# HikariTJU/LD

Measured on AMD Instinct MI355X. Metric: images/sec (1333x800) GFocal-R50<-R101 LD train step, higher is better.
Workload: dtype f32

## Files before the change

include/ld_hip.h:

```cpp
#ifndef LD_HIP_H_
#define LD_HIP_H_

#include <stddef.h>
#include <stdint.h>

#ifdef __cplusplus
extern "C" {
#endif

#define LD_MAX_LEVELS 8
#define LD_NUM_LOSS_KEYS 8

#define LD_EINVAL (-1)
#define LD_ENOSPACE (-2)
#define LD_EUNSUPPORTED (-3)

typedef void* ld_stream_t;

typedef struct {
  int32_t H, W;
  int32_t stride;
  int32_t offset;
} ld_level_t;

// ... 205 lines not shown
  void* y_raw_c8;
} ld_conv_epilogue_t;

size_t ld_conv_weight_image_floats(int Cout, int Cin, int KH, int KW,
                                   int backward);
int ld_conv_weight_transform(const float* w, int Cout, int Cin, int KH, int KW,
                             float* wt_fwd, float* wt_bwd, ld_stream_t stream);
typedef struct {
  const float* w;
  float* wt_fwd;
  float* wt_bwd;
  int32_t Cout, Cin, ntaps, first_block;
} ld_wt_job_t;
int ld_conv_weight_transform_batch(const ld_wt_job_t* jobs, const int32_t* block_job,
                                   int nblocks, ld_stream_t stream);
int ld_conv_weight_transform_tiles(int Cout, int Cin, int ntaps, int bf16);
int ld_conv_weight_transform_batch_tiled(const ld_wt_job_t* jobs,
                                         const int32_t* block_job, int nblocks, int bf16,
                                         ld_stream_t stream);
int ld_conv_forward(const ld_conv_t* c, const float* x, const float* wt_fwd,
                    const ld_conv_epilogue_t* ep, float* y, ld_stream_t stream);
int ld_conv_dgrad(const ld_conv_t* c, const float* dy, const float* wt_bwd,
                  float* dx, ld_stream_t stream);
int ld_conv_dgrad_acc(const ld_conv_t* c, const float* dy, const float* wt_bwd,
                      const float* addend, float* dx, ld_stream_t stream);
int ld_conv_tune_forward(const ld_conv_t* c, const float* x, const float* wt_fwd,
                         const ld_conv_epilogue_t* ep, float* y,
                         ld_stream_t stream);
int ld_conv_tune_dgrad(const ld_conv_t* c, const float* dy, const float* wt_bwd,
                       float* dx, ld_stream_t stream);
int ld_conv_tune_load(const char* path);
int ld_conv_tune_save(const char* path);
int ld_conv_tune_clear(void);
long long ld_conv_tune_hits(const int* key);
int ld_conv_tune_reset_hits(void);
size_t ld_conv_wgrad_workspace_bytes(const ld_conv_t* c);
size_t ld_conv_tune_wgrad_workspace_bytes(const ld_conv_t* c);
int ld_conv_wgrad(const ld_conv_t* c, const float* x, const float* dy, float* dw,
                  int accumulate, void* workspace, size_t workspace_bytes,
                  ld_stream_t stream);
typedef struct {
  const float* slabs;
  float* dw;
  int32_t splits, ntaps, Cout, Cin, accumulate, first_block;
} ld_wgrad_job_t;
int ld_conv_wgrad_partial(const ld_conv_t* c, int family, const void* x, const void* dy,
                          void* slabs, size_t slab_bytes, ld_wgrad_job_t* job,
                          ld_stream_t stream);
int ld_wgrad_reduce_batch(const ld_wgrad_job_t* jobs, const int32_t* block_job,
                          int nblocks, ld_stream_t stream);
int ld_conv_wgrad_plan(const ld_conv_t* c, int* out);
int ld_conv_tune_wgrad(const ld_conv_t* c, const float* x, const float* dy, float* dw,
                       void* workspace, size_t workspace_bytes, ld_stream_t stream);

size_t ld_conv_bf16_weight_image_elems(int Cout, int Cin, int KH, int KW,
                                       int backward);
int ld_conv_bf16_weight_transform(const float* w, int Cout, int Cin, int KH, int KW,
                                  void* wt_fwd, void* wt_bwd, ld_stream_t stream);
int ld_conv_bf16_weight_transform_batch(const ld_wt_job_t* jobs,
                                        const int32_t* block_job, int nblocks,
                                        ld_stream_t stream);
int ld_conv_bf16_forward(const ld_conv_t* c, const float* x, const void* wt_fwd,
                         const ld_conv_epilogue_t* ep, float* y, ld_stream_t stream);
int ld_conv_bf16_tune_forward(const ld_conv_t* c, const float* x, const void* wt_fwd,
                              const ld_conv_epilogue_t* ep, float* y,
                              ld_stream_t stream);
// ... 459 lines not shown
```

ld_amd/csrc/conv.hip:

```cpp
#include <hip/hip_runtime.h>
#include <type_traits>
#include <stdio.h>
#include <stdlib.h>

#include <mutex>
#include <string>
#include <unordered_map>
#include <vector>

#include "conv_common.h"
#include "conv_tune.h"

namespace {

template <int BM, int BNT, int BKT, int MODE, int KG, int WVM, int WVN>
__global__ __launch_bounds__(64 * WVM * WVN * KG) void conv_igemm_kernel(ConvK a) {
  constexpr int NT = 64 * WVM * WVN;
  constexpr int WM = BM / WVM, WN = BNT / WVN;
  constexpr int TM = WM / 32, TN = WN / 32;
  constexpr int A_PER = BKT * BM / NT;
  constexpr int B_PER = BKT * BNT / NT;
  static_assert(A_PER >= 1 && B_PER >= 1, "tile too small");
  constexpr int NBUF = 2;
  constexpr int GROUP_LDS = NBUF * BKT * (BM + BNT);
  constexpr int NACC = TM * TN * 16;
  static_assert(KG == 1 || (KG - 1) * NACC * NT <= KG * GROUP_LDS,
                "split-K reduction does not fit the tile LDS");
  __shared__ float lds[KG * GROUP_LDS + 2 * BM];
  const int kg = __builtin_amdgcn_readfirstlane((int)threadIdx.x / NT);
  float* As = lds + kg * GROUP_LDS;
  float* Bs = As + NBUF * BKT * BM;

  const int t = threadIdx.x % NT, lane = t & 63, wave = t >> 6;
  const int wm = wave / WVN, wn = wave % WVN;
  const int mtiles = (a.Cout + BM - 1) / BM;
  const int tile = xcd_swizzle(blockIdx.x, gridDim.x);
  const int m0 = (tile % mtiles) * BM;
// ... 276 lines not shown
      locate_out(a.g, p, l, hc, wc);
      p = a.foff[l] + (2 * hc + a.ph) * a.fW[l] + 2 * wc + a.pw;
      prow = a.Pfull;
    }
    const size_t colbase = (size_t)n * a.Cout * prow + p;
#pragma unroll
    for (int i = 0; i < TM; ++i) {
      const int rbase = wm * WM + i * 32 + 4 * lk;
      float res[16];
      if (has_res) {
#pragma unroll
        for (int r = 0; r < 16; ++r) {
          const int row = rbase + (r & 3) + 8 * (r >> 2);
          res[r] = (m0 + row < a.Cout)
                       ? a.residual[colbase + (size_t)(m0 + row) * prow]
                       : 0.0f;
        }
      }
#pragma unroll
      for (int r = 0; r < 16; ++r) {
        const int row = rbase + (r & 3) + 8 * (r >> 2);
        if (m0 + row >= a.Cout) continue;
        float v = acc[i][j][r] * s_scale[row] + s_shift[row];
        if (MODE == 0 && a.y_raw)
          a.y_raw[colbase + (size_t)(m0 + row) * prow] = acc[i][j][r];
        if (has_res) v += res[r];
        if (relu) v = fmaxf(v, 0.0f);
        a.y[colbase + (size_t)(m0 + row) * prow] = v;
      }
    }
  }
}

template <int TM, int TN, int WVM, int MODE, int D, int OCC, int KS, int DBG = 0>
__global__ __launch_bounds__(256, OCC) void conv_stream_kernel(ConvK a) {
  static_assert(KS == 1 || (KS == 4 && WVM == 1), "KS is 1 or 4");
  static_assert(D * (TM + TN) < 64, "ring exceeds the 6-bit vmcnt counter");
  constexpr int WVN = 4 / WVM;
  constexpr int WM = TM * 32, WN = TN * 32;
  constexpr int BM = KS == 4 ? WM : WVM * WM, BNT = KS == 4 ? WN : WVN * WN;
  __shared__ float red[KS == 4 ? 2 * TM * TN * 16 * 64 : 1];
  const int lane = threadIdx.x & 63;
  const int wave = __builtin_amdgcn_readfirstlane((int)threadIdx.x >> 6);
  const int wm = KS == 4 ? 0 : wave / WVN, wn = KS == 4 ? 0 : wave % WVN;
  const int kslice = KS == 4 ? wave : 0;
  const int l31 = lane & 31, lk = lane >> 5;
  const int mtiles = (a.Cout + BM - 1) / BM;
  const int tile = xcd_swizzle(blockIdx.x, gridDim.x);
  const int m0 = (tile % mtiles) * BM + wm * WM;
  const int n0 = (tile / mtiles) * BNT + wn * WN;
  if (m0 >= a.Cout || n0 >= a.J) return;

  const int Cin = __builtin_amdgcn_readfirstlane(a.Cin);
  const int Cout = __builtin_amdgcn_readfirstlane(a.Cout);
  const int KW = __builtin_amdgcn_readfirstlane(a.KW);
  const int Pin = __builtin_amdgcn_readfirstlane(a.Pin);
  const int Kpad = __builtin_amdgcn_readfirstlane(a.Kpad);
  const int ntw = __builtin_amdgcn_readfirstlane(MODE == 1 ? a.ntw : a.KW);
  const int ntaps = __builtin_amdgcn_readfirstlane(
      MODE == 1 ? a.nth * a.ntw : a.KH * a.KW);

  int bHin[TN], bWin[TN], boff[TN], bh0[TN], bw0[TN];
#pragma unroll
  for (int j = 0; j < TN; ++j) {
    const int jb = n0 + j * 32 + l31;
    bHin[j] = 0;
    bWin[j] = 0;
    boff[j] = 0;
    bh0[j] = 0;
    bw0[j] = 0;
    if (jb < a.J) {
      const int n = jb / a.Pout, p = jb - n * a.Pout;
      int bl, bho, bwo;
      locate_out(a.g, p, bl, bho, bwo);
      bHin[j] = a.g.lv[bl].Hin;
      bWin[j] = a.g.lv[bl].Win;
      boff[j] = n * Cin * Pin + a.g.lv[bl].off_in + lk * Pin;
      if (MODE == 1) {
        bh0[j] = bho + a.ch0;
        bw0[j] = bwo + a.cw0;
      } else {
        bh0[j] = bho * a.g.stride - a.g.pad;
        bw0[j] = bwo * a.g.stride - a.g.pad;
// ... 185 lines not shown
            rv[j][e] = buf_load(r_res, ok ? voff[j] : kOOB, (unsigned)(rl + e) * prow4);
          }
      }
#pragma unroll
      for (int e = 0; e < 4; ++e) {
        const bool ok = m0 + 4 * lk + rl + e < Cout;
        const float scale = has_aff ? sc[e] : 1.0f;
        const float shift = sh[e] + bi[e];
        const unsigned so = (unsigned)(rl + e) * prow4;
#pragma unroll
        for (int j = 0; j < TN; ++j) {
          const int r = 4 * g + e;
          const unsigned vo = ok ? voff[j] : kOOB;
          const float av = acc[i][j][r];
          float v = av * scale + shift;
          if (RAW)
            __builtin_amdgcn_raw_buffer_store_b32(__builtin_bit_cast(unsigned, av), r_raw,
                                                  vo, so, 0);
          if (RES) v += rv[j][e];
          v = relu ? fmaxf(v, 0.0f) : v;
          __builtin_amdgcn_raw_buffer_store_b32(__builtin_bit_cast(unsigned, v), r_y, vo,
                                                so, 0);
        }
      }
    }
  };
  if (has_res) {
    if (has_raw) run(std::true_type{}, std::true_type{});
    else run(std::true_type{}, std::false_type{});
  } else {
    if (has_raw) run(std::false_type{}, std::true_type{});
    else run(std::false_type{}, std::false_type{});
  }
}

template <int VEC>
struct VecF;
template <>
struct VecF<2> { typedef float T __attribute__((ext_vector_type(2))); };
template <>
struct VecF<4> { typedef float T __attribute__((ext_vector_type(4))); };

template <int VEC>
__device__ __forceinline__ typename VecF<VEC>::T buf_load_vec(rsrc_t r, unsigned voff,
                                                             unsigned soff) {
  typedef typename VecF<VEC>::T V;
  if constexpr (VEC == 2)
    return __builtin_bit_cast(V, __builtin_amdgcn_raw_buffer_load_b64(r, voff, soff, 0));
  else
    return __builtin_bit_cast(V, __builtin_amdgcn_raw_buffer_load_b128(r, voff, soff, 0));
}

template <int TM, int VEC, int WVM, int D>
__global__ __launch_bounds__(256, 2) void conv1x1_vec_kernel(ConvK a) {
  static_assert(D * (TM + 1) < 64, "ring exceeds the 6-bit vmcnt counter");
  typedef typename VecF<VEC>::T V;
  constexpr int WVN = 4 / WVM;
  constexpr int WM = TM * 32, WN = VEC * 32;
  constexpr int BM = WVM * WM, BNT = WVN * WN;
  const int lane = threadIdx.x & 63;
  const int wave = __builtin_amdgcn_readfirstlane((int)threadIdx.x >> 6);
  const int wm = wave / WVN, wn = wave % WVN;
  const int l31 = lane & 31, lk = lane >> 5;
  const int mtiles = (a.Cout + BM - 1) / BM;
  const int tile = xcd_swizzle(blockIdx.x, gridDim.x);
  const int m0 = (tile % mtiles) * BM + wm * WM;
// ... 925 lines not shown
  }
  return LD_EUNSUPPORTED;
}

#define MODE1_TAPS(k) ((k).nth > 0 ? (k).nth * (k).ntw : (k).KH * (k).KW)
inline bool stream_cfg_fits(const ConvK& k, const StreamCfg& c) {
  if (c.wvm < 1) return false;
  if (k.Cin % (2 * c.d) != 0) return false;
  if (c.ks == 2) {
    if (k.KH != 1 || k.KW != 1 || k.g.stride != 1 || k.g.pad != 0 || k.nth > 0 ||
        k.Pin != k.Pout || k.Pout % c.tn != 0 || k.x_c8 || k.y_c8 || k.res_c8)
      return false;
    const uintptr_t m = (uintptr_t)(c.tn * 4 - 1);
    if ((((uintptr_t)k.x | (uintptr_t)k.y | (uintptr_t)k.residual |
          (uintptr_t)k.y_raw) & m) != 0)
      return false;
    const int bmv = c.wvm * c.tm * 32, cout32v = (k.Cout + 31) / 32 * 32;
    if (c.wvm > 1 && bmv > cout32v) return false;
    if (c.wvm == 1 && c.tm * 32 >= cout32v + 32) return false;
    return true;
  }
  if (c.d == 4 && k.Cin % 16 == 0) return false;
  const int bm = c.wvm * c.tm * 32;
  const int cout32 = (k.Cout + 31) / 32 * 32;
  if (c.ks == 4) {
    const int nchunks = (MODE1_TAPS(k)) * (k.Cin / (2 * c.d));
    if (nchunks < 16) return false;
  }
  if (c.wvm > 1 && bm > cout32) return false;
  if (c.wvm == 1 && c.tm * 32 >= cout32 + 32) return false;
  return true;
}

inline int stream_cfg_model(const ConvK& k) {
  int best = -1;
  double best_t = 0;
  for (int i = 0; i < kNumStreamCfgs; ++i) {
    const StreamCfg& c = kStreamCfgs[i];
    if (c.ks == 2) continue;
    if (!stream_cfg_fits(k, c)) continue;
    const int bm = (c.ks == 4 ? 1 : c.wvm) * c.tm * 32;
    const int bn = (c.ks == 4 ? 1 : 4 / c.wvm) * c.tn * 32;
    const long nb = (long)((k.Cout + bm - 1) / bm) * ((k.J + bn - 1) / bn);
    const int area = c.tm * c.tn;
    const double eff = (area >= 4 ? 0.90 : area >= 2 ? 0.84 : 0.79) *
                       (c.ks == 4 ? 0.97 : 1.0);
    const int occ = area >= 4 ? 4 : 5;
    const double rounds =
        nb <= 256L * occ ? (double)((nb + 255) / 256) : (double)nb / 256.0;
    const double t = rounds * (c.ks == 4 ? 1 : 4) * area / eff;
    if (best < 0 || t < best_t) {
      best = i;
      best_t = t;
    }
  }
  return best;
}

inline LdTuneCfg stream_cfg_rec(const StreamCfg& c) {
  return LdTuneCfg{c.tm, c.tn, c.wvm, c.d, c.ks};
}

template <int MODE>
int launch_stream(const ConvK& k, hipStream_t stream) {
  if (k.Cin % 8 != 0) return LD_EUNSUPPORTED;
  auto launch = [&](const StreamCfg& c, int cap) {
    return launch_stream_cfg<MODE>(k, c, stream, cap);
  };
  auto by_model = [&] {
    const int m = stream_cfg_model(k);
    return m < 0 ? LD_EUNSUPPORTED : launch(kStreamCfgs[m], 0);
  };
  auto forced = [&](int* rc) {
    const char* env = getenv("LD_CONV_STREAM");
    if (!env) return false;
    *rc = LD_EUNSUPPORTED;
    if (env[0] == '0' && env[1] == 0) return true;
    StreamCfg c;
    c.ks = 1;
    int cap = 0;
    if (sscanf(env, "%dx%dx%dx%dx%dx%d", &c.tm, &c.tn, &c.wvm, &c.d, &c.ks, &cap) < 4)
      return false;
    while (c.d > 4 && k.Cin % (2 * c.d) != 0) c.d /= 2;
    if (!(c.ks == 2 && !stream_cfg_fits(k, c))) {
      *rc = launch(c, cap);
      if (*rc != LD_EUNSUPPORTED) return true;
      c.ks = 1;
      *rc = launch(c, cap);
      if (*rc != LD_EUNSUPPORTED) return true;
    }
    *rc = by_model();
    return true;
  };
  return launch_picked(MODE, 0, k, kStreamCfgs, forced, stream_cfg_rec, stream_cfg_fits,
                       stream_cfg_model, launch);
}

template <int MODE>
int tune_stream(const ConvK& k, hipStream_t stream) {
  if (k.Cin % 8 != 0) return 1;
  const LdTuneKey key = make_tune_key(MODE, 0, k);
  if (int r = tune_refused(key, stream)) return r;
  int pick = stream_cfg_model(k);
  if (pick < 0) return 1;
  TuneTimer timer(stream);
  float best_ms = -1.0f;
  int best_cap = 0;
  static const int kCaps[] = {0, 4, 3, 2};
  for (int i = 0; i < kNumStreamCfgs; ++i) {
    if (!stream_cfg_fits(k, kStreamCfgs[i])) continue;
    for (const int cap_try : kCaps) {
      const float ms = timer.time(
          [&] { return launch_stream_cfg<MODE>(k, kStreamCfgs[i], stream, cap_try); });
      if (ms == TuneTimer::kLaunchFailed) break;
      if (ms < 0.0f) continue;
      if (best_ms < 0.0f || ms < best_ms * (cap_try ? 0.99f : 1.0f)) {
        best_ms = ms;
        pick = i;
        best_cap = cap_try;
      }
    }
  }
  const StreamCfg& c = kStreamCfgs[pick];
  if (tune_log_level() == 1) {
    const double fl = 2.0 * k.J * k.Cout * k.Cin *
                      (MODE == 1 ? k.nth * k.ntw : k.KH * k.KW);
    fprintf(stderr,
            "[ld_conv] mode %d Cin %d Cout %d k %dx%d s%d J %d lv %d -> "
            "%dx%dx%dx%dx%d cap %d  %.1f TFLOP/s\n",
            MODE, k.Cin, k.Cout, k.KH, k.KW, k.g.stride, k.J, k.g.num_levels,
            c.tm, c.tn, c.wvm, c.d, c.ks, best_cap, tune_tflops(fl, best_ms));
  }
  if (best_ms > 0.0f) {
    LdTuneCfg rec = stream_cfg_rec(c);
    rec.cap = best_cap;
    ld_tune_store(key, rec);
  }
  return 0;
}

template <int MODE>
int launch_igemm(const ConvK& k_in, hipStream_t stream) {
  ConvK k = k_in;
  k.pipe = 1;
  if (const char* env = getenv("LD_CONV_PIPE")) k.pipe = atoi(env) != 0;
  if constexpr (MODE != 2) {
    const int rc = launch_stream<MODE>(k, stream);
    if (rc != LD_EUNSUPPORTED) return rc;
  }
  const TileCfg c = pick_tile(k);
  const int nb = tile_blocks(k, c);
  int kgroups = 1;
  if (c.bm == 64 && c.bn == 64 && MODE != 2) {
    const int ksteps = ((k.Cin + c.bk - 1) / c.bk) * k.KH * k.KW;
    if (nb < 400 && ksteps >= 8) kgroups = 2;
// ... 79 lines not shown
  if (g_tune.find(k) == g_tune.end()) return -1;
  auto it = g_tune_hits.find(k);
  return it == g_tune_hits.end() ? 0 : it->second;
}

extern "C" int ld_conv_tune_reset_hits(void) {
  std::lock_guard<std::mutex> lock(g_tune_mu);
  g_tune_hits.clear();
  return 0;
}

void ld_tune_store(const LdTuneKey& key, const LdTuneCfg& cfg) {
  std::lock_guard<std::mutex> lock(g_tune_mu);
  g_tune[key] = cfg;
}

extern "C" int ld_conv_tune_load(const char* path) {
  if (!path || !*path) return LD_EINVAL;
  FILE* f = fopen(path, "r");
  if (!f) return LD_EINVAL;
  int n = 0;
  char line[1024];
  while (fgets(line, sizeof(line), f)) {
    if (line[0] == '#' || line[0] == '\n') continue;
    LdTuneKey k;
    LdTuneCfg c;
    int pos = 0, adv = 0, got = 0;
    for (int i = 0; i < 18; ++i)
      if (sscanf(line + pos, "%d%n", &k.v[i], &adv) == 1) {
        pos += adv;
        ++got;
      }
    c.cap = 0;
    if (got == 18 && sscanf(line + pos, "%d %d %d %d %d %d", &c.tm, &c.tn, &c.wvm, &c.d,
                            &c.ks, &c.cap) >= 5) {
      ld_tune_store(k, c);
      ++n;
    }
  }
  fclose(f);
  return n;
}

extern "C" int ld_conv_tune_save(const char* path) {
  if (!path || !*path) return LD_EINVAL;
  FILE* f = fopen(path, "w");
  if (!f) return LD_EINVAL;
  std::lock_guard<std::mutex> lock(g_tune_mu);
  fprintf(f, "# ld_amd conv shape table: MODE Cin Cout KH KW stride pad J levels Hin0 "
             "Win0 ph pw relu res affine family 0 | tm tn wvm d ks cap\n");
  for (const auto& kv : g_tune) {
    for (int i = 0; i < 18; ++i) fprintf(f, "%d ", kv.first.v[i]);
    fprintf(f, " %d %d %d %d %d %d\n", kv.second.tm, kv.second.tn, kv.second.wvm,
            kv.second.d, kv.second.ks, kv.second.cap);
  }
  fclose(f);
  return (int)g_tune.size();
}

extern "C" int ld_conv_tune_clear(void) {
  std::lock_guard<std::mutex> lock(g_tune_mu);
  g_tune.clear();
  return 0;
}

extern "C" size_t ld_conv_weight_image_floats(int Cout, int Cin, int KH, int KW,
                                             int backward) {
  if (Cout < 1 || Cin < 1 || KH < 1 || KW < 1) return 0;
  return backward ? (size_t)KH * KW * kpad_rows(Cout) * Cin
                  : (size_t)KH * KW * kpad_rows(Cin) * Cout;
}

extern "C" int ld_conv_weight_transform(const float* w, int Cout, int Cin, int KH,
                                        int KW, float* wt_fwd, float* wt_bwd,
                                        ld_stream_t stream) {
  if (!w || Cout < 1 || Cin < 1 || KH < 1 || KW < 1 || (!wt_fwd && !wt_bwd))
    return LD_EINVAL;
  const int cip = kpad_rows(Cin), cop = kpad_rows(Cout);
  size_t total = 0;
  if (wt_fwd) total = (size_t)KH * KW * cip * Cout;
  if (wt_bwd) total = max(total, (size_t)KH * KW * cop * Cin);
  LD_LAUNCH(conv_weight_transform_kernel,
                     dim3((unsigned)((total + 255) / 256)), dim3(256), 0,
                     (hipStream_t)stream, w, Cout, Cin, KH * KW, cip, cop, wt_fwd,
                     wt_bwd);
  return (int)hipGetLastError();
}

extern "C" int ld_conv_weight_transform_batch(const ld_wt_job_t* jobs,
                                              const int32_t* block_job, int nblocks,
                                              ld_stream_t stream) {
  if (!jobs || !block_job || nblocks < 1) return LD_EINVAL;
  LD_LAUNCH(conv_weight_transform_batch_kernel, dim3(nblocks), dim3(256), 0,
                     (hipStream_t)stream, jobs, block_job);
  return (int)hipGetLastError();
// ... 763 lines not shown
```

ld_amd/csrc/conv_common.h:

```cpp
#pragma once
#include <hip/hip_runtime.h>
#include <stdint.h>

#include "../../include/ld_hip.h"
#include "ld_launch.h"

struct Geo {
  int stride, pad, num_levels;
  ld_conv_level_t lv[LD_MAX_LEVELS];
};

struct ConvK {
  const float* x;
  const float* wt;
  float* y;
  const float* bias;
  const float* scale;
  const float* shift;
  const float* residual;
  int relu;
  int N, Cin, Cout, KH, KW;
  int Pin, Pout;
  int J;
  int Kpad;
// ... 89 lines not shown
    if (i < a.num_levels && p >= a.lv[i].off_out) l = i;
  const int r = p - a.lv[l].off_out;
  ho = r / a.lv[l].Wout;
  wo = r - ho * a.lv[l].Wout;
}

template <int MODE>
__device__ __forceinline__ bool tap_offset(const Geo& a, int l, int ho, int wo,
                                           int kh, int kw, int& off) {
  const int Hin = a.lv[l].Hin, Win = a.lv[l].Win;
  int hi, wi;
  if (MODE == 0) {
    hi = ho * a.stride - a.pad + kh;
    wi = wo * a.stride - a.pad + kw;
  } else {
    const int hn = ho - a.pad + kh, wn = wo - a.pad + kw;
    if ((hn | wn) < 0 || ((hn | wn) & 1)) return false;
    hi = hn >> 1;
    wi = wn >> 1;
  }
  if (hi < 0 || hi >= Hin || wi < 0 || wi >= Win) return false;
  off = a.lv[l].off_in + hi * Win + wi;
  return true;
}

}

struct LdTuneKey {
  int v[18];
};
struct LdTuneCfg {
  int tm, tn, wvm, d, ks;
  int cap = 0;
};
bool ld_tune_lookup(const LdTuneKey& key, LdTuneCfg* out);
void ld_tune_store(const LdTuneKey& key, const LdTuneCfg& cfg);

namespace {
inline LdTuneKey make_tune_key(int mode, int family, const ConvK& k) {
  static const bool resc8 = [] {
    const char* e = getenv("LD_TUNE_KEY_RESC8");
    return !(e && e[0] == '0');
  }();
  const bool res = k.residual != nullptr || (resc8 && k.res_c8 != nullptr);
  return LdTuneKey{{mode, k.Cin, k.Cout, k.KH, k.KW, k.g.stride, k.g.pad, k.J,
                    k.g.num_levels, k.g.lv[0].Hin, k.g.lv[0].Win, k.ph, k.pw, k.relu,
                    res && !k.tune_plain, k.scale != nullptr, family, 0}};
}
}
```

ld_amd/csrc/conv_tune.h:

```cpp
#pragma once
#include <stdlib.h>

#include "conv_common.h"

namespace {
constexpr int kTuneReps = 3;

inline int tune_log_level() {
  const char* lg = getenv("LD_CONV_TUNE_LOG");
  return lg && (lg[0] == '1' || lg[0] == '2') ? lg[0] - '0' : 0;
}

inline double tune_tflops(double flop, float best_ms) {
  return best_ms > 0 ? flop / (best_ms * 1e-3 / kTuneReps) / 1e12 : 0.0;
}

inline int tune_refused(const LdTuneKey& key, hipStream_t stream) {
  LdTuneCfg have;
  if (ld_tune_lookup(key, &have)) return 1;
  hipStreamCaptureStatus cap = hipStreamCaptureStatusNone;
  (void)hipStreamIsCapturing(stream, &cap);
  return cap != hipStreamCaptureStatusNone ? LD_EUNSUPPORTED : 0;
}

class TuneTimer {
 public:
  static constexpr float kLaunchFailed = -2.0f;

  explicit TuneTimer(hipStream_t stream) : stream_(stream) {
    (void)hipDeviceSynchronize();
    (void)hipEventCreate(&e0_);
    (void)hipEventCreate(&e1_);
  }
  ~TuneTimer() {
// ... 14 lines not shown
      (void)hipEventElapsedTime(&t, e0_, e1_);
      if (ms < 0.0f || t < ms) ms = t;
    }
    return ms;
  }

 private:
  hipStream_t stream_;
  hipEvent_t e0_, e1_;
};

template <class Cfg, int N, class Rec>
int tune_cfg_index(const Cfg (&tab)[N], const LdTuneCfg& t, Rec rec, bool cap_is_shape) {
  for (int i = 0; i < N; ++i) {
    const LdTuneCfg r = rec(tab[i]);
    if (r.tm == t.tm && r.tn == t.tn && r.wvm == t.wvm && r.d == t.d && r.ks == t.ks &&
        (!cap_is_shape || r.cap == t.cap))
      return i;
  }
  return -1;
}

template <class Cfg, int N, class Forced, class Rec, class Fits, class Model, class Launch>
int launch_picked(int mode, int family, const ConvK& k, const Cfg (&tab)[N], Forced forced,
                  Rec rec, Fits fits, Model model, Launch launch) {
  int rc = 0;
  if (forced(&rc)) return rc;
  int pick = -1;
  LdTuneCfg t;
  if (ld_tune_lookup(make_tune_key(mode, family, k), &t)) {
    pick = tune_cfg_index(tab, t, rec, family == 2);
    if (pick >= 0 && !fits(k, tab[pick])) pick = -1;
  }
  const int cap = pick >= 0 ? t.cap : 0;
  if (pick < 0) pick = model(k);
  if (pick < 0) return LD_EUNSUPPORTED;
  return launch(tab[pick], cap);
}
}
```

ld_amd/lib.py:

```python
import ctypes as C
import os

import torch

_HERE = os.path.dirname(os.path.abspath(__file__))
LIB_PATH = os.path.join(_HERE, '_lib', 'libldhip.so')

LD_MAX_LEVELS = 8
LD_NUM_LOSS_KEYS = 8
LD_SGD_MAX_CLASSES = 64
LOSS_KEYS = ('loss_cls', 'loss_bbox', 'loss_dfl', 'loss_ld', 'loss_ld_vlr',
             'loss_kd', 'loss_kd_neg', 'loss_im')


class LdError(RuntimeError):
    pass


class LevelT(C.Structure):
    _fields_ = [('H', C.c_int32), ('W', C.c_int32), ('stride', C.c_int32),
                ('offset', C.c_int32)]


class GeomT(C.Structure):
# ... 165 lines not shown
                ('y_raw', C.c_void_p), ('y_raw_c8', C.c_void_p)]


class LevelsT(C.Structure):
    _fields_ = [('num_levels', C.c_int32), ('H', C.c_int32 * LD_MAX_LEVELS),
                ('W', C.c_int32 * LD_MAX_LEVELS)]


_lib = None


def lib_available():
    return os.path.exists(LIB_PATH)


def get_lib():
    global _lib
    if _lib is not None:
        return _lib
    if not os.path.exists(LIB_PATH):
        raise LdError(
            f'{LIB_PATH} not found: the HIP extension has not been built '
            '(run `python -m ld_amd.build`); ld_amd has no fallback path')
    lib = C.CDLL(LIB_PATH)
    _declare(lib)
    if lib.ld_abi_version() != ABI_VERSION:
        raise LdError('libldhip.so ABI version mismatch; rebuild')
    _load_tune_tables(lib)
    _lib = lib
    return lib


TUNE_TABLE = os.path.join(_HERE, 'tune', 'gfx950.txt')


def _load_tune_tables(lib):
    if os.environ.get('LD_CONV_TUNE_TABLE', '1') != '0' and \
            os.path.exists(TUNE_TABLE):
        lib.ld_conv_tune_load(TUNE_TABLE.encode())
    extra = os.environ.get('LD_CONV_TUNE_FILE')
    if extra and os.path.exists(extra):
        lib.ld_conv_tune_load(extra.encode())


def save_tune_table(path):
    return get_lib().ld_conv_tune_save(str(path).encode())


ABI_VERSION = 16
_vp, _i64, _i32, _f32, _sz = C.c_void_p, C.c_int64, C.c_int, C.c_float, C.c_size_t
_G, _H, _M = C.POINTER(GeomT), C.POINTER(LossHpT), C.POINTER(MapsT)
_CV, _EP, _LV = C.POINTER(ConvT), C.POINTER(ConvEpilogueT), C.POINTER(LevelsT)
_AV = C.POINTER(AugViewT)

SIGNATURES = {
    'ld_abi_version': (C.c_int, []),
    'ld_target_arch': (C.c_char_p, []),
    'ld_atss_targets_workspace_bytes': (_sz, [_G, _i32]),
    'ld_atss_targets': (C.c_int, [_G, _H, _vp, _vp, _vp, _i32, _vp, _vp, _vp,
                                  _vp, _vp, _vp, _vp, _vp, _sz, _vp]),
    'ld_atss_targets_ex': (C.c_int, [_G, _H, _vp, _vp, _vp, _vp, _i32, _vp,
                                     _vp, _vp, _vp, _vp, _vp, _vp, _vp, _vp,
                                     _vp, _sz, _vp]),
    'ld_grid_anchors': (C.c_int, [_G, _vp, _vp]),
    'ld_loss_workspace_bytes': (_sz, [_G]),
    'ld_fcos_targets': (C.c_int, [_G, _i32, C.POINTER(C.c_float), _i32, _f32,
                                  _vp, _vp, _vp, _i32, _vp, _vp, _vp, _vp, _vp,
                                  _vp, _vp]),
    'ld_retina_targets_workspace_bytes': (_sz, [_G, _i32, _i32]),
    'ld_retina_targets': (C.c_int, [_G, _i32, _vp, _i32, _f32, _f32, _f32, _i32,
                                    _vp, _vp, _vp, _i32, _vp, _vp, _vp, _vp,
                                    _vp, _vp, _vp, _vp, _vp, _sz, _vp]),
# ... 143 lines not shown
    'ld_conv_bf16_tune_forward': (C.c_int, [_CV, _vp, _vp, _EP, _vp, _vp]),
    'ld_conv_bf16_dgrad': (C.c_int, [_CV, _vp, _vp, _vp, _vp]),
    'ld_conv_bf16_dgrad_acc': (C.c_int, [_CV, _vp, _vp, _vp, _vp, _vp]),
    'ld_conv_bf16_tune_dgrad': (C.c_int, [_CV, _vp, _vp, _vp, _vp]),
    'ld_conv_bf16_wgrad': (C.c_int, [_CV, _vp, _vp, _vp, _i32, _vp, _sz,
                                     _vp]),
    'ld_conv_bf16_wgrad_c8': (C.c_int, [_CV, _vp, _vp, _vp, _i32, _vp, _sz,
                                        _vp]),
    'ld_conv_to_c8': (C.c_int, [_vp, _i32, _i32, _i32, _vp, _vp]),
    'ld_conv_bf16_forward_c8': (C.c_int, [_CV, _vp, _vp, _EP, _vp, _vp]),
    'ld_conv_bf16_tune_forward_c8': (C.c_int, [_CV, _vp, _vp, _EP, _vp, _vp]),
    'ld_conv_bf16_dgrad_c8': (C.c_int, [_CV, _vp, _vp, _vp, _vp]),
    'ld_conv_bf16_dgrad_c8_acc': (C.c_int, [_CV, _vp, _vp, _vp, _vp, _vp]),
    'ld_record_begin': (C.c_int, []),
    'ld_record_end': (C.c_int64, []),
    'ld_record_abort': (C.c_int, []),
    'ld_record_count': (C.c_int, [C.c_int64]),
    'ld_record_replay': (C.c_int, [C.c_int64, _vp]),
    'ld_record_free': (C.c_int, [C.c_int64]),
    'ld_stream_fork': (C.c_int, [_vp, _vp]),
    'ld_step_list_build': (C.c_int64, [_vp, _i32]),
    'ld_copy_d2d': (C.c_int, [_vp, _vp, _sz, _vp]),
    'ld_step_list_info': (C.c_int, [C.c_int64, C.POINTER(C.c_int)]),
    'ld_step_list_replay': (C.c_int, [C.c_int64, _vp]),
    'ld_step_list_free': (C.c_int, [C.c_int64]),
    'ld_step_list_last_failure': (C.c_int, [C.POINTER(C.c_int)]),
    'ld_bottleneck_c8_supported': (C.c_int, [_i32, _i32, _i32, _i32]),
    'ld_bottleneck_c8_forward': (C.c_int, [C.POINTER(BottleneckT), _vp, _vp,
                                           _vp]),
    'ld_conv_bf16_tune_dgrad_c8': (C.c_int, [_CV, _vp, _vp, _vp, _vp]),
    'ld_conv_tune_load': (C.c_int, [C.c_char_p]),
    'ld_conv_tune_save': (C.c_int, [C.c_char_p]),
    'ld_conv_tune_clear': (C.c_int, []),
    'ld_conv_tune_hits': (C.c_longlong, [C.POINTER(C.c_int32)]),
    'ld_conv_tune_reset_hits': (C.c_int, []),
    'ld_conv_wgrad_workspace_bytes': (_sz, [_CV]),
    'ld_conv_wgrad_partial': (C.c_int, [_CV, _i32, _vp, _vp, _vp, _sz,
                                        C.POINTER(WgradJobT), _vp]),
    'ld_wgrad_reduce_batch': (C.c_int, [_vp, _vp, _i32, _vp]),
    'ld_bn_act_backward_nsplit': (C.c_int, [_i32, _i32, _i32, _i32]),
    'ld_bias_grad_nsplit': (C.c_int, [_i32, _i32, _i32]),
    'ld_bias_grad_partial': (C.c_int, [_vp, _i32, _i32, _i32, _vp, _sz, _vp]),
    'ld_bn_bwd_finalize_batch': (C.c_int, [_vp, _vp, _i32, _vp]),
    'ld_conv_tune_wgrad_workspace_bytes': (_sz, [_CV]),
    'ld_conv_wgrad': (C.c_int, [_CV, _vp, _vp, _vp, _i32, _vp, _sz, _vp]),
    'ld_conv_tune_wgrad': (C.c_int, [_CV, _vp, _vp, _vp, _vp, _sz, _vp]),
    'ld_conv_wgrad_plan': (C.c_int, [_CV, C.POINTER(C.c_int)]),
    'ld_bn_prepare': (C.c_int, [_vp, _vp, _vp, _vp, _f32, _i32, _vp, _vp, _vp,
                                _vp]),
    'ld_bn_act_forward_c8': (C.c_int, [_vp, _vp, _vp, _vp, _i32, _i32, _i32,
                                       _i32, _vp, _vp, _vp]),
    'ld_bn_act_forward': (C.c_int, [_vp, _vp, _vp, _vp, _i32, _i32, _i32,
                                    _i32, _vp, _vp]),
    'ld_bn_act_backward_workspace_bytes': (_sz, [_i32, _i32, _i32]),
    'ld_bn_act_backward': (C.c_int, [_vp, _vp, _vp, _vp, _vp, _vp, _i32, _i32,
                                     _i32, _i32, _vp, _vp, _vp, _vp, _i32,
                                     _vp, _sz, _vp]),
    'ld_bn_act_backward_c8': (C.c_int, [_vp, _vp, _vp, _vp, _vp, _vp, _i32,
                                        _i32, _i32, _i32, _vp, _vp, _vp, _vp,
                                        _vp, _i32, _vp, _sz, _vp]),
    'ld_bn_act_backward_c8in': (C.c_int, [_vp, _vp, _vp, _vp, _vp, _vp, _i32,
                                          _i32, _i32, _i32, _vp, _vp, _vp, _vp,
                                          _vp, _i32, _vp, _sz, _vp]),
    'ld_bias_grad': (C.c_int, [_vp, _i32, _i32, _i32, _vp, _i32, _vp]),
    'ld_gn_forward_workspace_bytes': (_sz, [_LV, _i32, _i32]),
    'ld_gn_forward': (C.c_int, [_LV, _vp, _vp, _vp, _i32, _i32, _i32, _f32,
# ... 154 lines not shown
```

Measured before the change: 58.78.

## Add mixed-tile stream conv kernel covering bulk and tail columns in one launch

Adds a conv_stream_mixed_kernel in which the first blocks run a large bulk tile shape over the leading columns and the remaining blocks run a smaller tail tile over the leftover columns. The split point is derived from CU count and residency so the bulk covers whole waves. This is meant to reduce the partial last wave (tail effect) of forward convolutions. It also adds tuner support, an optional mixed tune table file, and extended table records. Whether it runs depends on tune table entries (gfx950_mixed.txt) or on tuning being enabled, which makes the gain shape-dependent.

```diff
diff --git a/include/ld_hip.h b/include/ld_hip.h
--- a/include/ld_hip.h
+++ b/include/ld_hip.h
@@ -261,6 +261,9 @@
 int ld_conv_tune_load(const char* path);
 int ld_conv_tune_save(const char* path);
 int ld_conv_tune_clear(void);
+int ld_conv_stream_pair_check(const int* bulk, const int* tail, int Cout, int J, int jb,
+                              int* grid);
+long long ld_conv_stream_mixed_launches(void);
 long long ld_conv_tune_hits(const int* key);
 int ld_conv_tune_reset_hits(void);
 size_t ld_conv_wgrad_workspace_bytes(const ld_conv_t* c);
diff --git a/ld_amd/csrc/conv.hip b/ld_amd/csrc/conv.hip
--- a/ld_amd/csrc/conv.hip
+++ b/ld_amd/csrc/conv.hip
@@ -2,7 +2,9 @@
 #include <type_traits>
 #include <stdio.h>
 #include <stdlib.h>
-
+#include <string.h>
+
+#include <atomic>
 #include <mutex>
 #include <string>
 #include <unordered_map>
@@ -345,23 +347,23 @@
   }
 }
 
-template <int TM, int TN, int WVM, int MODE, int D, int OCC, int KS, int DBG = 0>
-__global__ __launch_bounds__(256, OCC) void conv_stream_kernel(ConvK a) {
+template <int TM, int TN, int WVM, int MODE, int D, int KS, int DBG>
+__device__ __forceinline__ void conv_stream_body(const ConvK& a, float* red, int b, int nb,
+                                                 int j0) {
   static_assert(KS == 1 || (KS == 4 && WVM == 1), "KS is 1 or 4");
   static_assert(D * (TM + TN) < 64, "ring exceeds the 6-bit vmcnt counter");
   constexpr int WVN = 4 / WVM;
   constexpr int WM = TM * 32, WN = TN * 32;
   constexpr int BM = KS == 4 ? WM : WVM * WM, BNT = KS == 4 ? WN : WVN * WN;
-  __shared__ float red[KS == 4 ? 2 * TM * TN * 16 * 64 : 1];
   const int lane = threadIdx.x & 63;
   const int wave = __builtin_amdgcn_readfirstlane((int)threadIdx.x >> 6);
   const int wm = KS == 4 ? 0 : wave / WVN, wn = KS == 4 ? 0 : wave % WVN;
   const int kslice = KS == 4 ? wave : 0;
   const int l31 = lane & 31, lk = lane >> 5;
   const int mtiles = (a.Cout + BM - 1) / BM;
-  const int tile = xcd_swizzle(blockIdx.x, gridDim.x);
+  const int tile = xcd_swizzle(b, nb);
   const int m0 = (tile % mtiles) * BM + wm * WM;
-  const int n0 = (tile / mtiles) * BNT + wn * WN;
+  const int n0 = j0 + (tile / mtiles) * BNT + wn * WN;
   if (m0 >= a.Cout || n0 >= a.J) return;
 
   const int Cin = __builtin_amdgcn_readfirstlane(a.Cin);
@@ -613,6 +615,25 @@
     if (has_raw) run(std::false_type{}, std::true_type{});
     else run(std::false_type{}, std::false_type{});
   }
+}
+
+template <int TM, int TN, int WVM, int MODE, int D, int OCC, int KS, int DBG = 0>
+__global__ __launch_bounds__(256, OCC) void conv_stream_kernel(ConvK a) {
+  __shared__ float red[KS == 4 ? 2 * TM * TN * 16 * 64 : 1];
+  conv_stream_body<TM, TN, WVM, MODE, D, KS, DBG>(a, red, blockIdx.x, gridDim.x, 0);
+}
+
+template <int TM, int TN, int WVM, int D, int TM2, int TN2, int WVM2, int D2, int KS>
+__global__ __launch_bounds__(256, KS == 4 ? 4 : 2) void conv_stream_mixed_kernel(
+    ConvK a, int nb_bulk, int jb) {
+  constexpr int AREA = TM * TN > TM2 * TN2 ? TM * TN : TM2 * TN2;
+  __shared__ float red[KS == 4 ? 2 * AREA * 16 * 64 : 1];
+  const int b = blockIdx.x;
+  if (b < nb_bulk)
+    conv_stream_body<TM, TN, WVM, 0, D, KS, 0>(a, red, b, nb_bulk, 0);
+  else
+    conv_stream_body<TM2, TN2, WVM2, 0, D2, KS, 0>(a, red, b - nb_bulk,
+                                                   (int)gridDim.x - nb_bulk, jb);
 }
 
 template <int VEC>
@@ -1604,6 +1625,97 @@
   return true;
 }
 
+#define LD_MIX_PAIRS(X)                                                            \
+  X(2, 1, 1, 16, 1, 1, 1, 16, 4) X(1, 2, 1, 16, 1, 1, 1, 16, 4)                    \
+  X(2, 1, 1, 8, 1, 1, 1, 8, 4) X(2, 2, 1, 8, 1, 1, 1, 8, 4)                        \
+  X(3, 1, 1, 8, 1, 1, 4, 8, 1) X(2, 2, 2, 8, 1, 1, 4, 8, 1)                        \
+  X(3, 2, 1, 8, 1, 1, 1, 8, 1)
+struct MixCfg {
+  StreamCfg bulk, tail;
+};
+constexpr MixCfg kMixCfgs[] = {
+#define LD_MIX_ROW(TM_, TN_, WVM_, D_, TM2_, TN2_, WVM2_, D2_, KS_)                \
+  {{TM_, TN_, WVM_, D_, KS_}, {TM2_, TN2_, WVM2_, D2_, KS_}},
+    LD_MIX_PAIRS(LD_MIX_ROW)
+#undef LD_MIX_ROW
+};
+constexpr int kNumMixCfgs = sizeof(kMixCfgs) / sizeof(kMixCfgs[0]);
+
+inline bool stream_pair_ok(const StreamCfg& b, const StreamCfg& t) {
+  if (b.ks != t.ks || (b.ks != 1 && b.ks != 4)) return false;
+  if (b.ks == 4 && b.d != t.d) return false;
+  return true;
+}
+
+inline void stream_block(const StreamCfg& c, int& bm, int& bn) {
+  bm = (c.ks == 4 ? 1 : c.wvm) * c.tm * 32;
+  bn = (c.ks == 4 ? 1 : 4 / c.wvm) * c.tn * 32;
+}
+
+struct MixGrid {
+  int nb_bulk, nb_tail, jb;
+};
+inline MixGrid mix_grid(const ConvK& k, const StreamCfg& b, const StreamCfg& t, int jb) {
+  int bm, bn, tm, tn;
+  stream_block(b, bm, bn);
+  stream_block(t, tm, tn);
+  const int mt_b = (k.Cout + bm - 1) / bm, mt_t = (k.Cout + tm - 1) / tm;
+  MixGrid g;
+  if (jb >= k.J) {
+    g.jb = k.J;
+    g.nb_bulk = mt_b * ((k.J + bn - 1) / bn);
+    g.nb_tail = 0;
+  } else {
+    g.jb = jb > 0 ? jb / bn * bn : 0;
+    g.nb_bulk = mt_b * (g.jb / bn);
+    g.nb_tail = mt_t * ((k.J - g.jb + tn - 1) / tn);
+  }
+  return g;
+}
+
+std::atomic<long long> g_mixed_launches{0};
+
+inline int launch_stream_mixed(const ConvK& k, const StreamCfg& b, const StreamCfg& t, int jb,
+                               hipStream_t stream, int cap, int* residency = nullptr) {
+  if (!stream_pair_ok(b, t)) return LD_EUNSUPPORTED;
+  if (b.d < 1 || t.d < 1 || k.Cin % (2 * b.d) != 0 || k.Cin % (2 * t.d) != 0)
+    return LD_EUNSUPPORTED;
+  if (k.nth > 0) return LD_EUNSUPPORTED;
+  const MixGrid g = mix_grid(k, b, t, jb);
+  const int area = max(b.tm * b.tn, t.tm * t.tn);
+  const unsigned lds = cap_lds_bytes(cap, b.ks == 4 ? 2 * area * 16 * 64 * 4 : 4);
+#define LD_MIX_CASE(TM_, TN_, WVM_, D_, TM2_, TN2_, WVM2_, D2_, KS_)                     \
+  if (b.tm == TM_ && b.tn == TN_ && b.wvm == WVM_ && b.d == D_ && t.tm == TM2_ &&        \
+      t.tn == TN2_ && t.wvm == WVM2_ && t.d == D2_ && b.ks == KS_) {                     \
+    auto kern = conv_stream_mixed_kernel<TM_, TN_, WVM_, D_, TM2_, TN2_, WVM2_, D2_, KS_>; \
+    if (residency)                                                                       \
+      return (int)hipOccupancyMaxActiveBlocksPerMultiprocessor(residency, kern, 256, lds); \
+    LD_LAUNCH(kern, dim3(g.nb_bulk + g.nb_tail), dim3(256), lds, stream, k, g.nb_bulk,   \
+              g.jb);                                                                     \
+    ++g_mixed_launches;                                                                  \
+    return (int)hipGetLastError();                                                       \
+  }
+  LD_MIX_PAIRS(LD_MIX_CASE)
+#undef LD_MIX_CASE
+  return LD_EUNSUPPORTED;
+}
+
+inline int mix_split(const ConvK& k, const StreamCfg& b, const StreamCfg& t, int cap,
+                     bool per_cu = false) {
+  int res = 0, dev = 0, cus = 0;
+  if (launch_stream_mixed(k, b, t, 0, nullptr, cap, &res) != 0 || res < 1) return -1;
+  if (hipGetDevice(&dev) != hipSuccess ||
+      hipDeviceGetAttribute(&cus, hipDeviceAttributeMultiprocessorCount, dev) != hipSuccess ||
+      cus < 1)
+    return -1;
+  int bm, bn;
+  stream_block(b, bm, bn);
+  const long slots = (long)cus * (per_cu ? 1 : res);
+  const long mt = (k.Cout + bm - 1) / bm, ct = (k.J + bn - 1) / bn;
+  const long rounds = mt * ct / slots;
+  return (int)(rounds * slots / mt) * bn;
+}
+
 inline int stream_cfg_model(const ConvK& k) {
   int best = -1;
   double best_t = 0;
@@ -1639,6 +1751,14 @@
   auto launch = [&](const StreamCfg& c, int cap) {
     return launch_stream_cfg<MODE>(k, c, stream, cap);
   };
+  auto launch_rec = [&](const StreamCfg& c, const LdTuneCfg& t) {
+    if (MODE == 0 && t.t_tm > 0) {
+      const StreamCfg tail{t.t_tm, t.t_tn, t.t_wvm, t.t_d, t.t_ks};
+      const int rc = launch_stream_mixed(k, c, tail, t.jb, stream, t.cap);
+      if (rc != LD_EUNSUPPORTED) return rc;
+    }
+    return launch(c, t.cap);
+  };
   auto by_model = [&] {
     const int m = stream_cfg_model(k);
     return m < 0 ? LD_EUNSUPPORTED : launch(kStreamCfgs[m], 0);
@@ -1654,6 +1774,19 @@
     if (sscanf(env, "%dx%dx%dx%dx%dx%d", &c.tm, &c.tn, &c.wvm, &c.d, &c.ks, &cap) < 4)
       return false;
     while (c.d > 4 && k.Cin % (2 * c.d) != 0) c.d /= 2;
+    if (const char* plus = strchr(env, '+')) {
+      StreamCfg t;
+      t.ks = 1;
+      int jb = 0;
+      const char* at = strchr(plus, '@');
+      if (MODE == 0 && at &&
+          sscanf(plus + 1, "%dx%dx%dx%dx%d", &t.tm, &t.tn, &t.wvm, &t.d, &t.ks) >= 4 &&
+          sscanf(at + 1, "%d", &jb) == 1) {
+        while (t.d > 4 && k.Cin % (2 * t.d) != 0) t.d /= 2;
+        *rc = launch_stream_mixed(k, c, t, jb, stream, cap);
+        if (*rc != LD_EUNSUPPORTED) return true;
+      }
+    }
     if (!(c.ks == 2 && !stream_cfg_fits(k, c))) {
       *rc = launch(c, cap);
       if (*rc != LD_EUNSUPPORTED) return true;
@@ -1665,13 +1798,129 @@
     return true;
   };
   return launch_picked(MODE, 0, k, kStreamCfgs, forced, stream_cfg_rec, stream_cfg_fits,
-                       stream_cfg_model, launch);
+                       stream_cfg_model, launch_rec);
+}
+
+struct MixPick {
+  int pair = -1, jb = 0, cap = 0;
+};
+
+inline void tune_mixes(const ConvK& k, hipStream_t stream, TuneTimer& timer, int ks, int d,
+                       int cap_extra, float margin, float* best_ms, MixPick* pick) {
+  for (int p = 0; p < kNumMixCfgs; ++p) {
+    const StreamCfg &b = kMixCfgs[p].bulk, &t = kMixCfgs[p].tail;
+    if (ks && (b.ks != ks || (ks == 4 && b.d != d))) continue;
+    if (!stream_cfg_fits(k, b) || !stream_cfg_fits(k, t)) continue;
+    int bm, bn;
+    stream_block(b, bm, bn);
+    const int caps[] = {0, 4, 3, 2, cap_extra};
+    for (int ci = 0; ci < (cap_extra > 4 ? 5 : 4); ++ci) {
+      const int cap = caps[ci];
+      int jbs[6], njb = 0;
+      for (int per_cu = 0; per_cu < 2; ++per_cu) {
+        const int jb0 = mix_split(k, b, t, cap, per_cu != 0);
+        for (int s = -1; s <= 1 && jb0 >= 0; ++s) {
+          const int jb = jb0 + s * bn;
+          bool seen = jb <= 0 || jb >= k.J;
+          for (int i = 0; i < njb; ++i) seen |= jbs[i] == jb;
+          if (!seen) jbs[njb++] = jb;
+        }
+      }
+      for (int ji = 0; ji < njb; ++ji) {
+        const int jb = jbs[ji];
+        const float ms = timer.time(
+            [&] { return launch_stream_mixed(k, b, t, jb, stream, cap); });
+        if (tune_log_level() == 1)
+          fprintf(stderr, "[ld_conv]   mix %dx%dx%dx%d + %dx%dx%dx%d ks %d jb %d cap %d  %.4f ms\n",
+                  b.tm, b.tn, b.wvm, b.d, t.tm, t.tn, t.wvm, t.d, b.ks, jb, cap,
+                  ms / kTuneReps);
+        if (ms > 0.0f && (*best_ms < 0.0f || ms < *best_ms * margin)) {
+          *best_ms = ms;
+          pick->pair = p;
+          pick->jb = jb;
+          pick->cap = cap;
+        }
+      }
+    }
+  }
+}
+
+inline LdTuneCfg mix_rec(const MixPick& m) {
+  const StreamCfg &b = kMixCfgs[m.pair].bulk, &t = kMixCfgs[m.pair].tail;
+  LdTuneCfg rec{b.tm, b.tn, b.wvm, b.d, b.ks};
+  rec.cap = m.cap;
+  rec.t_tm = t.tm, rec.t_tn = t.tn, rec.t_wvm = t.wvm, rec.t_d = t.d, rec.t_ks = t.ks;
+  rec.jb = m.jb;
+  return rec;
+}
+
+inline int retune_stream_mixed(const ConvK& k, const LdTuneKey& key, const LdTuneCfg& have,
+                               hipStream_t stream) {
+  if (have.ks != 1 && have.ks != 4) return 1;
+  hipStreamCaptureStatus capturing = hipStreamCaptureStatusNone;
+  (void)hipStreamIsCapturing(stream, &capturing);
+  if (capturing != hipStreamCaptureStatusNone) return LD_EUNSUPPORTED;
+  const StreamCfg cur{have.tm, have.tn, have.wvm, have.d, have.ks};
+  TuneTimer timer(stream);
+  const float base_ms =
+      timer.time([&] { return launch_stream_cfg<0>(k, cur, stream, have.cap); });
+  if (base_ms <= 0.0f) return 1;
+  float best_ms = base_ms;
+  int uni = -1;
+  for (int i = 0; i < kNumStreamCfgs; ++i) {
+    const StreamCfg& c = kStreamCfgs[i];
+    if (c.ks != have.ks || (c.ks == 4 && c.d != have.d) || !stream_cfg_fits(k, c)) continue;
+    bool in_pair = false;
+    for (int p = 0; p < kNumMixCfgs; ++p)
+      for (const StreamCfg* q : {&kMixCfgs[p].bulk, &kMixCfgs[p].tail})
+        in_pair |= q->tm == c.tm && q->tn == c.tn && q->wvm == c.wvm && q->d == c.d &&
+                   q->ks == c.ks;
+    if (!in_pair) continue;
+    const float ms = timer.time([&] { return launch_stream_cfg<0>(k, c, stream, 0); });
+    if (ms > 0.0f && ms < best_ms * 0.98f) {
+      best_ms = ms;
+      uni = i;
+    }
+  }
+  MixPick mix;
+  float mix_ms = uni >= 0 ? best_ms * 0.99f / 0.98f : base_ms;
+  tune_mixes(k, stream, timer, have.ks, have.d, have.cap, 0.98f, &mix_ms, &mix);
+  if (tune_log_level() == 1) {
+    const double fl = 2.0 * k.J * k.Cout * k.Cin * k.KH * k.KW;
+    fprintf(stderr,
+            "[ld_conv] mix-retune Cin %d Cout %d k %dx%d s%d J %d res %d: record "
+            "%dx%dx%dx%dx%d cap %d %.1f TFLOP/s",
+            k.Cin, k.Cout, k.KH, k.KW, k.g.stride, k.J, key.v[14], have.tm, have.tn, have.wvm,
+            have.d, have.ks, have.cap, tune_tflops(fl, base_ms));
+    if (mix.pair >= 0) {
+      const LdTuneCfg r = mix_rec(mix);
+      fprintf(stderr, " -> mix %dx%dx%dx%d + %dx%dx%dx%d jb %d cap %d %.1f TFLOP/s\n", r.tm,
+              r.tn, r.wvm, r.d, r.t_tm, r.t_tn, r.t_wvm, r.t_d, r.jb, r.cap,
+              tune_tflops(fl, mix_ms));
+    } else if (uni >= 0) {
+      const StreamCfg& c = kStreamCfgs[uni];
+      fprintf(stderr, " -> kept (one shape %dx%dx%dx%dx%d %.1f TFLOP/s, no mix faster)\n", c.tm,
+              c.tn, c.wvm, c.d, c.ks, tune_tflops(fl, best_ms));
+    } else {
+      fprintf(stderr, " -> kept (no mix faster)\n");
+    }
+  }
+  if (mix.pair >= 0) ld_tune_store(key, mix_rec(mix));
+  return 0;
 }
 
 template <int MODE>
 int tune_stream(const ConvK& k, hipStream_t stream) {
   if (k.Cin % 8 != 0) return 1;
   const LdTuneKey key = make_tune_key(MODE, 0, k);
+  if constexpr (MODE == 0) {
+    const char* env = getenv("LD_CONV_TUNE_MIX");
+    LdTuneCfg have;
+    if (env && env[0] == '1' && ld_tune_lookup(key, &have)) {
+      if (have.t_tm > 0) return 1;
+      return retune_stream_mixed(k, key, have, stream);
+    }
+  }
   if (int r = tune_refused(key, stream)) return r;
   int pick = stream_cfg_model(k);
   if (pick < 0) return 1;
@@ -1693,6 +1942,22 @@
       }
     }
   }
+  if constexpr (MODE == 0) {
+    MixPick mix;
+    float mix_ms = best_ms;
+    if (best_ms > 0.0f) tune_mixes(k, stream, timer, 0, 0, 0, 0.99f, &mix_ms, &mix);
+    if (mix.pair >= 0) {
+      const LdTuneCfg rec = mix_rec(mix);
+      if (tune_log_level() == 1)
+        fprintf(stderr,
+                "[ld_conv] mode 0 Cin %d Cout %d k %dx%d s%d J %d lv %d -> mix "
+                "%dx%dx%dx%d + %dx%dx%dx%d ks %d jb %d\n",
+                k.Cin, k.Cout, k.KH, k.KW, k.g.stride, k.J, k.g.num_levels, rec.tm, rec.tn,
+                rec.wvm, rec.d, rec.t_tm, rec.t_tn, rec.t_wvm, rec.t_d, rec.ks, rec.jb);
+      ld_tune_store(key, rec);
+      return 0;
+    }
+  }
   const StreamCfg& c = kStreamCfgs[pick];
   if (tune_log_level() == 1) {
     const double fl = 2.0 * k.J * k.Cout * k.Cin *
@@ -1838,8 +2103,11 @@
         ++got;
       }
     c.cap = 0;
-    if (got == 18 && sscanf(line + pos, "%d %d %d %d %d %d", &c.tm, &c.tn, &c.wvm, &c.d,
-                            &c.ks, &c.cap) >= 5) {
+    int nf = 0;
+    if (got == 18 && (nf = sscanf(line + pos, "%d %d %d %d %d %d %d %d %d %d %d %d", &c.tm,
+                                  &c.tn, &c.wvm, &c.d, &c.ks, &c.cap, &c.t_tm, &c.t_tn,
+                                  &c.t_wvm, &c.t_d, &c.t_ks, &c.jb)) >= 5) {
+      if (nf < 12) c.t_tm = c.t_tn = c.t_wvm = c.t_d = c.t_ks = c.jb = 0;
       ld_tune_store(k, c);
       ++n;
     }
@@ -1854,11 +2122,16 @@
   if (!f) return LD_EINVAL;
   std::lock_guard<std::mutex> lock(g_tune_mu);
   fprintf(f, "# ld_amd conv shape table: MODE Cin Cout KH KW stride pad J levels Hin0 "
-             "Win0 ph pw relu res affine family 0 | tm tn wvm d ks cap\n");
+             "Win0 ph pw relu res affine family 0 | tm tn wvm d ks cap "
+             "[tail tm tn wvm d ks, bulk columns]\n");
   for (const auto& kv : g_tune) {
     for (int i = 0; i < 18; ++i) fprintf(f, "%d ", kv.first.v[i]);
-    fprintf(f, " %d %d %d %d %d %d\n", kv.second.tm, kv.second.tn, kv.second.wvm,
+    fprintf(f, " %d %d %d %d %d %d", kv.second.tm, kv.second.tn, kv.second.wvm,
             kv.second.d, kv.second.ks, kv.second.cap);
+    if (kv.second.t_tm > 0)
+      fprintf(f, "  %d %d %d %d %d %d", kv.second.t_tm, kv.second.t_tn, kv.second.t_wvm,
+              kv.second.t_d, kv.second.t_ks, kv.second.jb);
+    fprintf(f, "\n");
   }
   fclose(f);
   return (int)g_tune.size();
@@ -1867,6 +2140,33 @@
 extern "C" int ld_conv_tune_clear(void) {
   std::lock_guard<std::mutex> lock(g_tune_mu);
   g_tune.clear();
+  return 0;
+}
+
+extern "C" long long ld_conv_stream_mixed_launches(void) { return g_mixed_launches.load(); }
+
+extern "C" int ld_conv_stream_pair_check(const int* bulk, const int* tail, int Cout, int J,
+                                         int jb, int* grid) {
+  if (!bulk || !tail) return LD_EINVAL;
+  const StreamCfg b{bulk[0], bulk[1], bulk[2], bulk[3], bulk[4]};
+  const StreamCfg t{tail[0], tail[1], tail[2], tail[3], tail[4]};
+  if (!stream_pair_ok(b, t)) return LD_EUNSUPPORTED;
+  bool have = false;
+  for (int p = 0; p < kNumMixCfgs; ++p) {
+    const StreamCfg &pb = kMixCfgs[p].bulk, &pt = kMixCfgs[p].tail;
+    have |= pb.tm == b.tm && pb.tn == b.tn && pb.wvm == b.wvm && pb.d == b.d &&
+            pb.ks == b.ks && pt.tm == t.tm && pt.tn == t.tn && pt.wvm == t.wvm &&
+            pt.d == t.d;
+  }
+  if (!have) return LD_EUNSUPPORTED;
+  if (grid) {
+    if (Cout < 1 || J < 1) return LD_EINVAL;
+    ConvK k{};
+    k.Cout = Cout;
+    k.J = J;
+    const MixGrid g = mix_grid(k, b, t, jb);
+    grid[0] = g.nb_bulk, grid[1] = g.nb_tail, grid[2] = g.jb;
+  }
   return 0;
 }
 
diff --git a/ld_amd/csrc/conv_common.h b/ld_amd/csrc/conv_common.h
--- a/ld_amd/csrc/conv_common.h
+++ b/ld_amd/csrc/conv_common.h
@@ -145,6 +145,7 @@
 struct LdTuneCfg {
   int tm, tn, wvm, d, ks;
   int cap = 0;
+  int t_tm = 0, t_tn = 0, t_wvm = 0, t_d = 0, t_ks = 0, jb = 0;
 };
 bool ld_tune_lookup(const LdTuneKey& key, LdTuneCfg* out);
 void ld_tune_store(const LdTuneKey& key, const LdTuneCfg& cfg);
diff --git a/ld_amd/csrc/conv_tune.h b/ld_amd/csrc/conv_tune.h
--- a/ld_amd/csrc/conv_tune.h
+++ b/ld_amd/csrc/conv_tune.h
@@ -1,5 +1,7 @@
 #pragma once
 #include <stdlib.h>
+
+#include <type_traits>
 
 #include "conv_common.h"
 
@@ -80,9 +82,12 @@
     pick = tune_cfg_index(tab, t, rec, family == 2);
     if (pick >= 0 && !fits(k, tab[pick])) pick = -1;
   }
-  const int cap = pick >= 0 ? t.cap : 0;
+  const bool tuned = pick >= 0;
   if (pick < 0) pick = model(k);
   if (pick < 0) return LD_EUNSUPPORTED;
-  return launch(tab[pick], cap);
+  if constexpr (std::is_invocable_v<Launch, const Cfg&, const LdTuneCfg&>)
+    return launch(tab[pick], tuned ? t : rec(tab[pick]));
+  else
+    return launch(tab[pick], tuned ? t.cap : 0);
 }
 }
diff --git a/ld_amd/lib.py b/ld_amd/lib.py
--- a/ld_amd/lib.py
+++ b/ld_amd/lib.py
@@ -221,12 +221,15 @@
 
 
 TUNE_TABLE = os.path.join(_HERE, 'tune', 'gfx950.txt')
+TUNE_TABLE_MIXED = os.path.join(_HERE, 'tune', 'gfx950_mixed.txt')
 
 
 def _load_tune_tables(lib):
     if os.environ.get('LD_CONV_TUNE_TABLE', '1') != '0' and \
             os.path.exists(TUNE_TABLE):
         lib.ld_conv_tune_load(TUNE_TABLE.encode())
+        if os.path.exists(TUNE_TABLE_MIXED):
+            lib.ld_conv_tune_load(TUNE_TABLE_MIXED.encode())
     extra = os.environ.get('LD_CONV_TUNE_FILE')
     if extra and os.path.exists(extra):
         lib.ld_conv_tune_load(extra.encode())
@@ -436,6 +439,10 @@
     'ld_conv_tune_load': (C.c_int, [C.c_char_p]),
     'ld_conv_tune_save': (C.c_int, [C.c_char_p]),
     'ld_conv_tune_clear': (C.c_int, []),
+    'ld_conv_stream_mixed_launches': (C.c_longlong, []),
+    'ld_conv_stream_pair_check': (C.c_int, [C.POINTER(C.c_int32), C.POINTER(C.c_int32),
+                                            C.c_int, C.c_int, C.c_int,
+                                            C.POINTER(C.c_int32)]),
     'ld_conv_tune_hits': (C.c_longlong, [C.POINTER(C.c_int32)]),
     'ld_conv_tune_reset_hits': (C.c_int, []),
     'ld_conv_wgrad_workspace_bytes': (_sz, [_CV]),
```

After: 59.54 (median of 4 runs). +1.3%, better.
